# gnns4hri/3D_multi_pose_estimator

Measured on AMD Instinct MI355X. Metric: frames/sec (5-view Panoptic, 4 persons) at 1/2/4/8 GPUs; MPJPE vs ref, higher is better.
Workload: dtype f32

## Files before the change

### 3d_multi_pose_estimator_amd/csrc/api.hip

```cpp
#include <cmath>
#include <cstdarg>
#include <new>
#include <cstdio>
#include <cstdlib>
#include <cstring>

#include "mpe_internal.h"
#include "assign_int.h"

using namespace mpe;

namespace {

int fail(mpe_ctx *ctx, int code, const char *fmt, ...) {
    char buf[512];
    va_list ap;
    va_start(ap, fmt);
    vsnprintf(buf, sizeof buf, fmt, ap);
    va_end(ap);
    if (ctx) ctx->err = buf;
    return code;
}

#define HIPCHK(ctx, expr)                                                                     \
// ... 362 lines not shown
    const int V = ctx->cfg.n_cameras, J = ctx->cfg.n_joints, npj = ctx->cfg.numbers_per_joint;
    if (ctx->mlp[0].in_dim != V * J * npj)
        return fail(ctx, MPE_ERR_INVALID, "MLP input width %d != V*J*numbers_per_joint = %d", ctx->mlp[0].in_dim,
                    V * J * npj);
    int widest = 0;
    for (int l = 0; l < ctx->mlp_layers; ++l) {
        if (l > 0 && ctx->mlp[l].in_dim != ctx->mlp[l - 1].out_dim)
            return fail(ctx, MPE_ERR_INVALID, "MLP layer %d input width mismatch", l);
        widest = widest > ctx->mlp[l].out_dim ? widest : ctx->mlp[l].out_dim;
    }
    ctx->mlp_ld_in = round_up(ctx->mlp[0].in_dim, 128);
    ctx->mlp_ld_hidden = round_up(widest, 128);
    const size_t rows = (size_t)ctx->cfg.max_frames * ctx->cfg.max_persons_per_frame;
    int rc;
    if ((rc = dev_alloc(ctx, &ctx->mlp_rows, rows * ctx->mlp_ld_in))) return rc;
    for (int i = 0; i < 2; ++i)
        if ((rc = dev_alloc(ctx, &ctx->mlp_act[i], rows * ctx->mlp_ld_hidden))) return rc;
    ctx->mlp_ws_ready = true;
    return MPE_OK;
}

enum GatInput {
    GAT_IN_IMPLICIT,
    GAT_IN_DENSE0,
    GAT_IN_ACT
};

int gat_layer_linear(mpe_ctx *ctx, hipStream_t s, const mpe_batch *b, int l, GatInput in, AggArgs *a, int *n_rows_ft2) {
    GatLayer &g = ctx->gat[l];
    const int V = ctx->cfg.n_cameras, J = ctx->cfg.n_joints;
    const int n_nodes = b->n_heads + b->n_edge_nodes;
    const bool red = ctx->gat_reduced;
    const bool half_rows = red || ctx->gat_attn_fp16;
    const int ld_ft = half_rows ? 2 * ctx->act_ld : ctx->act_ld;
    int rc;
    const AttnCoef coef{g.attn_l, g.attn_r, ctx->a12, g.heads, g.out_dim};
    const bool no_epi = getenv("MPE_NO_COEF_EPILOGUE") != nullptr;
    const AttnCoef *cp = no_epi ? nullptr : &coef;
    bool done = false;
    if (in == GAT_IN_DENSE0) {
        if ((rc = gat_linear(ctx, s, ctx->xdense, ctx->feat_ld, g.fc1, ctx->hdense, ctx->feat_ld, n_nodes, nullptr,
                             true, ctx->gat_alpha, false)))
            return rc;
        if ((rc = gat_linear(ctx, s, ctx->hdense, ctx->feat_ld, g.fc2, ctx->act[2], ld_ft, n_nodes, nullptr, false,
                             0.f, half_rows, nullptr, nullptr, -1.0, cp, &done)))
            return rc;
        a->ft2 = ctx->act[2];
        *n_rows_ft2 = n_nodes;
    } else if (in == GAT_IN_IMPLICIT) {
        if (ctx->l0_grouped && !red && linear_uses_tile_kernel(b->n_heads, g.in_dim)) {
            GemmProf gp(ctx, s, 2.0 * b->n_heads * (double)g.in_dim * (J * 10), 0, 0);
            HIPCHK(ctx, launch_linear_grouped(s, ctx->xc, ctx->l0_ld, ctx->l0_w, ctx->l0_ld,
                                              (long)weight_rows(g.in_dim) * ctx->l0_ld, ctx->l0_b, ctx->h0, ctx->feat_ld,
                                              b->n_heads, ctx->cam_count, V, ctx->cam_list, ctx->cfg.max_heads, g.in_dim,
                                              ctx->l0_ld, true, ctx->gat_alpha, ctx->gat_acc64));
        } else if (ctx->l0_grouped) {
            const double flop_each = 2.0 * b->n_heads * (double)g.in_dim * (J * 10) / V;
            for (int c = 0; c < V; ++c)
                if ((rc = gat_linear(ctx, s, ctx->xc, ctx->l0_ld, ctx->l0_fc1[c], ctx->h0, ctx->feat_ld, b->n_heads,
                                     ctx->cam_count + c, true, ctx->gat_alpha, false,
                                     ctx->cam_list + (size_t)c * ctx->cfg.max_heads,
                                     ctx->cam_list + (size_t)c * ctx->cfg.max_heads, flop_each)))
                    return rc;
        } else if ((rc = gat_linear(ctx, s, ctx->x0, ctx->feat_ld, g.fc1, ctx->h0, ctx->feat_ld, b->n_heads, nullptr,
                                    true, ctx->gat_alpha, false)))
            return rc;
        if ((rc = gat_linear(ctx, s, ctx->h0, ctx->feat_ld, g.fc2, ctx->act[1], ld_ft, b->n_heads, nullptr, false,
                             0.f, half_rows, nullptr, nullptr, -1.0, cp, &done)))
            return rc;
        a->ft2 = ctx->act[1];
        *n_rows_ft2 = b->n_heads;
        a->en_const_ft2 = ctx->en0_ft2;
        a->en_const_a = ctx->en0_a;
    } else {
        if ((rc = gat_linear(ctx, s, ctx->act[0], ctx->act_ld, g.fc1, ctx->act[1], ctx->act_ld, n_nodes, nullptr,
                             true, ctx->gat_alpha, false)))
            return rc;
        if ((rc = gat_linear(ctx, s, ctx->act[1], ctx->act_ld, g.fc2, ctx->act[2], ld_ft, n_nodes, nullptr, false,
                             0.f, half_rows, nullptr, nullptr, -1.0, cp, &done)))
            return rc;
        a->ft2 = ctx->act[2];
        *n_rows_ft2 = n_nodes;
    }
    if (!done && cp && g.out_dim == 40 && !half_rows && ctx->gat_split && !red) {
        HIPCHK(ctx, launch_attn_coef(s, a->ft2, ld_ft, *n_rows_ft2, g.heads, g.out_dim, g.attn_l, g.attn_r, ctx->a12, 0));
        done = true;
    }
    a->a12_ready = done ? 1 : 0;
    return MPE_OK;
}

AggArgs gat_agg_args(const mpe_ctx *ctx, int l) {
    const GatLayer &g = ctx->gat[l];
    AggArgs a{};
    a.heads = g.heads;
    a.out_dim = g.out_dim;
    a.alpha = ctx->gat_alpha;
    a.out_slope = ctx->gat_hidden_slope;
    const bool half_rows = ctx->gat_reduced || ctx->gat_attn_fp16;
    a.ft_half = half_rows ? 1 : 0;
    a.ld = half_rows ? 2 * ctx->act_ld : ctx->act_ld;
    a.a12 = ctx->a12;
    return a;
}

void agg_scores_out(const mpe_ctx *ctx, AggArgs *a, float *d_scores_en, float *d_scores_heads) {
    a->out_mode = ctx->gat_out_mode;
    a->score_mode = 1;
    a->out = d_scores_en;
    a->out_heads = d_scores_heads;
    a->ld_out = 1;
}

int gat_attention(mpe_ctx *ctx, hipStream_t s, const mpe_batch *b, int l, const AggArgs &a, int n_rows_ft2) {
    const GatLayer &g = ctx->gat[l];
    HIPCHK(ctx, launch_gat_attention(s, *b, ctx->cfg.n_cameras, ctx->cfg.max_heads_per_frame, ctx->node_off,
                                     ctx->head_frame, ctx->en_frame, ctx->en_pair, g.attn_l, g.attn_r, ctx->a12, a,
                                     n_rows_ft2, ctx->head_src, explicit_deg_cap(ctx->cfg.max_heads_per_frame), ctx->x_m_cap));
    return MPE_OK;
}

int gat_topology(mpe_ctx *ctx, hipStream_t s, const mpe_batch *b) {
    if (b->d_en_pair && (size_t)b->n_frames * ctx->cfg.max_heads_per_frame * explicit_deg_cap(ctx->cfg.max_heads_per_frame) > ctx->head_src_cap)
        return fail(ctx, MPE_ERR_CAPACITY, "in-edge table too small for %d frames with explicit edge-node lists", b->n_frames);
    HIPCHK(ctx, launch_topology(s, *b, ctx->cfg.n_cameras, ctx->node_off, ctx->head_frame, ctx->en_frame, ctx->en_pair,
                                ctx->cfg.max_heads_per_frame, ctx->d_status, ctx->head_src,
                                explicit_deg_cap(ctx->cfg.max_heads_per_frame), ctx->x_m_cap));
    return MPE_OK;
}

constexpr int LAT_MAX_FRAMES = 16;
constexpr int LAT_MAX_NODES = 16384;

bool lat_gat_ok(mpe_ctx *ctx, const mpe_batch *b, bool dense_in) {
    if (!latency_path_on() || dense_in || b->d_en_pair || b->n_frames > LAT_MAX_FRAMES) return false;
    if (b->n_heads + b->n_edge_nodes > LAT_MAX_NODES || b->n_heads <= 0) return false;
    if (!ctx->gat_split || ctx->gat_acc64 || ctx->gat_reduced || ctx->gat_attn_fp16 || !ctx->l0_grouped) return false;
    if (getenv("MPE_NO_COEF_EPILOGUE") || getenv("MPE_GAT_ACC64_MINK") || getenv("MPE_SKINNY_WAVES") || getenv("MPE_GEMM_NARROW")) return false;
    if (!lat_l0a_available(ctx->cfg.n_joints, ctx->l0_ld)) return false;
    const GatLayer &g0 = ctx->gat[0];
    if (g0.out_dim != 40 || g0.in_dim <= 512) return false;
    for (int l = 1; l < ctx->gat_layers; ++l) {
        const GatLayer &g = ctx->gat[l];
        if (!lat_gemm_available(g.fc1.ldw, g.in_dim, false, 0) || !lat_gemm_available(g.fc2.ldw, g.heads * g.out_dim, true, g.out_dim)) return false;
        if (g.in_dim > 512) return false;
    }
    const size_t shm = (size_t)2 * ((size_t)16 * (ctx->cfg.max_heads_per_frame + 1) + (ctx->cfg.max_heads_per_frame + 1) + 1 +
                                    (size_t)(ctx->cfg.n_cameras + 1) * (ctx->cfg.n_cameras + 1)) * sizeof(float);
    return shm <= 40 * 1024;
}

int ensure_lat_workspace(mpe_ctx *ctx) {
    if (ctx->gat_pl[0]) return MPE_OK;
    ctx->lat_rows = ctx->max_nodes < LAT_MAX_NODES ? ctx->max_nodes : LAT_MAX_NODES;
    ctx->gat_pl_plane = (size_t)ctx->lat_rows * ctx->act_ld;
    int rc;
    for (int i = 0; i < 2; ++i)
        if ((rc = dev_alloc(ctx, &ctx->gat_pl[i], 3 * ctx->gat_pl_plane))) return rc;
    return MPE_OK;
}

struct LatTail {
    bool deferred = false;
    const float *ft2 = nullptr;
    int ld = 0;
    float alpha = 0.f, out_slope = 0.f;
    int out_mode = 0;
// ... 1601 lines not shown
```

### 3d_multi_pose_estimator_amd/csrc/gat.hip

```cpp
#include <cstdlib>

#include "mpe_internal.h"
#include "sb_common.h"

namespace mpe {

__device__ __forceinline__ void topology_body(int f, int n_frames, int V, const int32_t *__restrict__ head_off,
                                              const int32_t *__restrict__ en_off, const int32_t *__restrict__ slot_n,
                                              int32_t *__restrict__ node_off, int32_t *__restrict__ head_frame,
                                              int32_t *__restrict__ en_frame, int32_t *__restrict__ en_pair, int hmax,
                                              int32_t *__restrict__ status) {
    __shared__ int s_n[MPE_MAX_CAMERAS], s_start[MPE_MAX_CAMERAS];
    const int h0 = head_off[f], H = head_off[f + 1] - h0;
    const int e0 = en_off[f], M = en_off[f + 1] - e0;
    if (threadIdx.x == 0) {
        int acc = 0;
        for (int s = 0; s < V; ++s) {
            s_n[s] = slot_n[f * V + s];
            s_start[s] = acc;
            acc += s_n[s];
        }
        node_off[f] = h0 + e0;
        if (H > hmax && status) atomicOr(status, 1);
        if (f == n_frames - 1) node_off[n_frames] = head_off[n_frames] + en_off[n_frames];
    }
    __syncthreads();
    for (int i = threadIdx.x; i < H; i += blockDim.x) head_frame[h0 + i] = f;
    for (int i = threadIdx.x; i < M; i += blockDim.x) en_frame[e0 + i] = f;
    int base = 0;
    for (int a = 0; a < V; ++a)
        for (int b = a + 1; b < V; ++b) {
            const int na = s_n[a], nb = s_n[b], cnt = na * nb;
            for (int t = threadIdx.x; t < cnt; t += blockDim.x) {
                const int i = t / nb, j = t - i * nb;
                en_pair[2 * (size_t)(e0 + base + t) + 0] = s_start[a] + i;
                en_pair[2 * (size_t)(e0 + base + t) + 1] = s_start[b] + j;
            }
            base += cnt;
        }
}

__global__ void k_topology(int n_frames, int V, const int32_t *__restrict__ head_off,
                           const int32_t *__restrict__ en_off, const int32_t *__restrict__ slot_n,
                           int32_t *__restrict__ node_off, int32_t *__restrict__ head_frame,
                           int32_t *__restrict__ en_frame, int32_t *__restrict__ en_pair, int hmax,
                           int32_t *__restrict__ status) {
    topology_body(blockIdx.x, n_frames, V, head_off, en_off, slot_n, node_off, head_frame, en_frame, en_pair, hmax, status);
}

__global__ void k_head_sources(int V, int hmax, const int32_t *__restrict__ head_off,
                               const int32_t *__restrict__ slot_n, uint16_t *__restrict__ head_src);

size_t head_src_entries(int max_heads_per_frame, int V) {
    const size_t h = (size_t)max_heads_per_frame;
    const size_t nodes = h + h * h * (size_t)(V - 1) / (2 * (size_t)V) + 1;
    return nodes <= 65535 ? h * (h + 1) : 0;
}

constexpr int XT_CHUNK = 2048;
__global__ __launch_bounds__(256) void k_topology_explicit(int n_frames, const int32_t *__restrict__ head_off,
                                                           const int32_t *__restrict__ en_off,
                                                           const int32_t *__restrict__ pairs_in,
                                                           int32_t *__restrict__ node_off, int32_t *__restrict__ head_frame,
                                                           int32_t *__restrict__ en_frame, int32_t *__restrict__ en_pair,
                                                           uint16_t *__restrict__ head_src, int hmax, int deg_cap, int m_cap,
                                                           int32_t *__restrict__ status) {
    __shared__ uint32_t s_pr[XT_CHUNK];
    const int f = blockIdx.x, t = threadIdx.x;
    const int h0 = head_off[f], H = head_off[f + 1] - h0;
    const int e0 = en_off[f], M = en_off[f + 1] - e0;
    const bool ok = H <= hmax && M <= m_cap;
    if (t == 0) {
        node_off[f] = h0 + e0;
        if (f == n_frames - 1) node_off[n_frames] = head_off[n_frames] + en_off[n_frames];
        if (!ok && status) atomicOr(status, 1);
    }
    for (int i = t; i < H; i += blockDim.x) head_frame[h0 + i] = f;
    int flag = 0;
    uint16_t *tab = head_src + (size_t)f * hmax * deg_cap;
    int deg_a[4];
#pragma unroll
    for (int r = 0; r < 4; ++r) {
        const int h = t + r * 256;
        deg_a[r] = 0;
// ... 605 lines not shown
            }
#pragma unroll
            for (int j = 0; j < 4; ++j)
#pragma unroll
                for (int k = 0; k < VEC; ++k) {
                    const float m = fv[j][k] * w[j];
                    acc[hf * 4 + j][k] = acc[hf * 4 + j][k] + m;
                }
        }
    }
#pragma unroll
    for (int j = 0; j < 8; ++j)
        if (e + j < deg) {
            float fv[VEC];
            row(e + j, fv);
            const float w = wt(e + j);
#pragma unroll
            for (int k = 0; k < VEC; ++k) {
                const float m = fv[k] * w;
                acc[j][k] = acc[j][k] + m;
            }
        }
#pragma unroll
    for (int k = 0; k < VEC; ++k)
        out[k] = ((acc[0][k] + acc[1][k]) + (acc[2][k] + acc[3][k])) + ((acc[4][k] + acc[5][k]) + (acc[6][k] + acc[7][k]));
}

constexpr int EN_ROWS = 16;

template <int VEC>
__device__ __forceinline__ void agg_store_row(const AggArgs &a, size_t row, int c, const float *o) {
    if (a.out_pl) {
        unsigned short *d = a.out_pl + row * a.ld_out + c;
        if (VEC == 4) {
            sb::f32x4 v = {o[0], o[1], o[2], o[3]};
            sb::store_planes4(d, a.out_pl_plane, v);
        } else {
#pragma unroll
            for (int k = 0; k < VEC; ++k) sb::store_planes1(d + k, a.out_pl_plane, o[k]);
        }
        return;
    }
    typedef float vecf __attribute__((ext_vector_type(VEC)));
    vecf v;
#pragma unroll
    for (int k = 0; k < VEC; ++k) v[k] = o[k];
    *reinterpret_cast<vecf *>(a.out + row * a.ld_out + c) = v;
}

__device__ __forceinline__ void row_coef(const float *__restrict__ fv, const AggArgs &a, int hh, float &x1, float &x2) {
    const float *al = a.attn_l + hh * a.out_dim, *ar = a.attn_r + hh * a.out_dim;
    if (a.out_dim == 40) {
        float v[40];
#pragma unroll
        for (int q = 0; q < 10; ++q) {
            const float4 x = *reinterpret_cast<const float4 *>(fv + 4 * q);
            v[4 * q] = x.x;
            v[4 * q + 1] = x.y;
            v[4 * q + 2] = x.z;
            v[4 * q + 3] = x.w;
        }
        coef40([&](int d) { return v[d]; }, al, ar, hh & 1, x1, x2);
    } else if (a.out_dim == 30) {
        float v[30];
#pragma unroll
        for (int q = 0; q < 15; ++q) {
            const float2 x = *reinterpret_cast<const float2 *>(fv + 2 * q);
            v[2 * q] = x.x;
            v[2 * q + 1] = x.y;
        }
        x1 = x2 = 0.f;
#pragma unroll
        for (int d = 0; d < 30; ++d) {
            x1 = __builtin_fmaf(v[d], al[d], x1);
            x2 = __builtin_fmaf(v[d], ar[d], x2);
        }
    } else {
        x1 = x2 = 0.f;
        for (int d = 0; d < a.out_dim; ++d) {
            x1 = __builtin_fmaf(fv[d], al[d], x1);
            x2 = __builtin_fmaf(fv[d], ar[d], x2);
        }
    }
}

template <int VEC, int ER = 16>
__device__ __forceinline__ void aggregate_en_body(int wg, int n_en, const int32_t *__restrict__ head_off,
                                                  const int32_t *__restrict__ en_off,
                                                  const int32_t *__restrict__ node_off,
                                                  const int32_t *__restrict__ en_frame,
                                                  const int32_t *__restrict__ en_pair, const AggArgs &a, int hmax) {
#pragma clang fp contract(off)
    __shared__ float s_w[ER][16][3];
    __shared__ int s_over[ER];
    __shared__ long s_src[ER][3];
    __shared__ long s_dst[ER];
    const int hd = a.heads * a.out_dim, heads = a.heads;
    const int per_row = (hd + VEC - 1) / VEC;
    const int m0 = wg * ER;
    const int rows = min(ER, n_en - m0);
    const bool l0 = a.en_const_ft2 != nullptr;
    for (int i = threadIdx.x; i < rows * heads; i += blockDim.x) {
        const int r = i / heads, hh = i - r * heads;
        const int m = m0 + r;
        const int f = en_frame[m];
        const int hb = head_off[f], H = head_off[f + 1] - hb;
        const int nb = node_off[f];
        const int v = H + (m - en_off[f]);
        const int h1 = en_pair[2 * (size_t)m], h2 = en_pair[2 * (size_t)m + 1];
        const float *ra1, *ra2, *ra3;
        if (l0) {
            ra1 = a.a12 + (size_t)(hb + h1) * 32;
            ra2 = a.a12 + (size_t)(hb + h2) * 32;
            ra3 = a.en_const_a;
        } else {
            ra1 = a.a12 + (size_t)(nb + h1) * 32;
            ra2 = a.a12 + (size_t)(nb + h2) * 32;
            ra3 = a.a12 + (size_t)(nb + v) * 32;
        }
        float a2v, c1, c2, c3;
        if (a.a12_ready) {
            a2v = ra3[16 + hh];
            c1 = ra1[hh];
            c2 = ra2[hh];
            c3 = ra3[hh];
        } else {
            const size_t rb = (size_t)(l0 ? hb : nb);
            float unused;
            row_coef(a.ft2 + (rb + h1) * a.ld + hh * a.out_dim, a, hh, c1, unused);
            row_coef(a.ft2 + (rb + h2) * a.ld + hh * a.out_dim, a, hh, c2, unused);
            if (l0) {
                c3 = a.en_const_a[hh];
                a2v = a.en_const_a[16 + hh];
            } else {
                row_coef(a.ft2 + (rb + v) * a.ld + hh * a.out_dim, a, hh, c3, a2v);
            }
        }
        float e1 = c1 + a2v, e2 = c2 + a2v, e3 = c3 + a2v;
        e1 = e1 > 0.f ? e1 : e1 * a.alpha;
        e2 = e2 > 0.f ? e2 : e2 * a.alpha;
        e3 = e3 > 0.f ? e3 : e3 * a.alpha;
        const float mx = fmaxf(fmaxf(e1, e2), e3);
        const float x1 = expf(e1 - mx), x2 = expf(e2 - mx), x3 = expf(e3 - mx);
        const float sum = (x1 + x2) + x3;
        s_w[r][hh][0] = x1 / sum;
        s_w[r][hh][1] = x2 / sum;
        s_w[r][hh][2] = x3 / sum;
        if (hh == 0) {
            s_src[r][0] = (long)(l0 ? hb : nb) + h1;
            s_src[r][1] = (long)(l0 ? hb : nb) + h2;
            s_src[r][2] = l0 ? -1 : (long)nb + v;
            s_dst[r] = (long)nb + v;
            s_over[r] = H > hmax ? 1 : 0;
        }
    }
    __syncthreads();
    for (int i = threadIdx.x; i < rows * per_row; i += blockDim.x) {
        const int r = i / per_row;
        const int c = (i - r * per_row) * VEC;
        const int hh = c / a.out_dim;
        float v1[VEC], v2[VEC], v3[VEC];
        ld_ftv<VEC>(a.ft2, (size_t)s_src[r][0] * a.ld + c, a.ft_half, v1);
        ld_ftv<VEC>(a.ft2, (size_t)s_src[r][1] * a.ld + c, a.ft_half, v2);
        if (l0) ld_ftv<VEC>(a.en_const_ft2, (size_t)c, 0, v3);
        else ld_ftv<VEC>(a.ft2, (size_t)s_src[r][2] * a.ld + c, a.ft_half, v3);
        float w1[VEC], w2[VEC], w3[VEC];
        const bool one_head = VEC == 1 || (c + VEC <= hd && (c + VEC - 1) / a.out_dim == hh);
#pragma unroll
        for (int k = 0; k < VEC; ++k) {
            int hk = hh;
            if (!one_head) {
                hk = (c + k) / a.out_dim;
                hk = hk < heads ? hk : heads - 1;
            }
            w1[k] = s_w[r][hk][0];
            w2[k] = s_w[r][hk][1];
            w3[k] = s_w[r][hk][2];
        }
        float o[VEC];
#pragma unroll
        for (int k = 0; k < VEC; ++k) {
            float acc = v1[k] * w1[k];
            acc = acc + v2[k] * w2[k];
            acc = acc + v3[k] * w3[k];
            o[k] = agg_activate(acc, a.out_mode, a.out_slope);
        }
        if (a.score_mode) a.out[m0 + r] = s_over[r] ? 0.f : o[0];
        else agg_store_row<VEC>(a, (size_t)s_dst[r], c, o);
    }
}

template <int VEC>
__global__ __launch_bounds__(256) void k_aggregate_en(int n_en, const int32_t *__restrict__ head_off,
                                                      const int32_t *__restrict__ en_off,
                                                      const int32_t *__restrict__ node_off,
                                                      const int32_t *__restrict__ en_frame,
                                                      const int32_t *__restrict__ en_pair, AggArgs a, int hmax) {
    aggregate_en_body<VEC, EN_ROWS>(blockIdx.x, n_en, head_off, en_off, node_off, en_frame, en_pair, a, hmax);
}

constexpr int AGG_ROWS = 2;

template <int VEC>
__device__ __forceinline__ void aggregate_heads_body(
    int wg, float *s_dyn, int n_heads, int V, int max_deg, const int32_t *__restrict__ head_off, const int32_t *__restrict__ en_off,
    const int32_t *__restrict__ slot_n, const int32_t *__restrict__ node_off,
    const int32_t *__restrict__ head_frame, const AggArgs &a, const uint16_t *__restrict__ head_src, int src_stride, int hmax) {
#pragma clang fp contract(off)
    const int heads = a.heads, hd = a.heads * a.out_dim;
    float *s_w = s_dyn;
    int *s_src = reinterpret_cast<int *>(s_w + (size_t)AGG_ROWS * heads * max_deg);
    int *s_topo = s_src + AGG_ROWS * max_deg;
    __shared__ int s_deg[AGG_ROWS], s_f[AGG_ROWS], s_v[AGG_ROWS], s_H[AGG_ROWS];

    const int t = threadIdx.x, lane = t & 63, wave = t >> 6;
    const bool l0 = a.en_const_ft2 != nullptr;
    const int r_own = wave & (AGG_ROWS - 1), half = wave / AGG_ROWS;
    const int gh = wg * AGG_ROWS + r_own;
    int deg = 0, f = 0, hb = 0, H = 0, v = 0;
    int32_t nb = 0;
    const int32_t *sn = slot_n;
    FrameTopo tp;
    tp.start = s_topo + r_own * (V + 1 + V * V);
    tp.base = tp.start + V + 1;
    bool live = false;
    if (gh < n_heads) {
        f = head_frame[gh];
        hb = head_off[f];
        H = head_off[f + 1] - hb;
        live = H <= hmax;
// ... 469 lines not shown
                    }
                    *reinterpret_cast<vecf *>(dst + 4 * g) = o;
                }
            } else {
                const int node = i / DV, d = (i - node * DV) * VEC;
                const int deg = s_deg[node];
                const int *src = s_src + node * max_deg;
                const float *w = s_wh + node * max_deg;
                float acc[VEC];
                weighted_sum8<VEC>(
                    deg,
                    [&](int e, float *fv) {
                        const vecf x = *reinterpret_cast<const vecf *>(s_ft + src[e] * Dp + d);
#pragma unroll
                        for (int k = 0; k < VEC; ++k) fv[k] = x[k];
                    },
                    [&](int e) { return w[e]; }, acc);
                vecf o;
#pragma unroll
                for (int k = 0; k < VEC; ++k) o[k] = agg_activate(acc[k], a.out_mode, a.out_slope);
                *reinterpret_cast<vecf *>(a.out + (size_t)(nb + node) * a.ld_out + c0 + d) = o;
            }
        }
        FUSED_STAMP(3);
        return;
    }
    for (int i = first * DV + t; i < N * DV; i += blockDim.x) {
        const int node = i / DV, d = (i - node * DV) * VEC;
        vecf o;
        if (node >= H) {
            const int m = node - H;
            const int pr = s_pair[m];
            const int h1 = pr >> 16, h2 = pr & 0xFFFF;
            const float w1 = s_wen[m * 3 + 0], w2 = s_wen[m * 3 + 1], w3 = s_wen[m * 3 + 2];
            const vecf f1 = *reinterpret_cast<const vecf *>(s_ft + h1 * Dp + d);
            const vecf f2 = *reinterpret_cast<const vecf *>(s_ft + h2 * Dp + d);
            const vecf f3 = *reinterpret_cast<const vecf *>(s_ft + node * Dp + d);
#pragma unroll
            for (int k = 0; k < VEC; ++k) {
                float acc = f1[k] * w1;
                acc = acc + f2[k] * w2;
                acc = acc + f3[k] * w3;
                o[k] = agg_activate(acc, a.out_mode, a.out_slope);
            }
        } else {
            const int deg = s_deg[node];
            const int *src = s_src + node * max_deg;
            const float *w = s_wh + node * max_deg;
            float acc[VEC];
            weighted_sum8<VEC>(
                deg,
                [&](int e, float *fv) {
                    const vecf x = *reinterpret_cast<const vecf *>(s_ft + src[e] * Dp + d);
#pragma unroll
                    for (int k = 0; k < VEC; ++k) fv[k] = x[k];
                },
                [&](int e) { return w[e]; }, acc);
#pragma unroll
            for (int k = 0; k < VEC; ++k) o[k] = agg_activate(acc[k], a.out_mode, a.out_slope);
        }
        if (a.score_mode) {
            if (node >= H) a.out[(size_t)eb + (node - H)] = o[0];
            else a.out_heads[(size_t)hb + node] = o[0];
        } else {
            *reinterpret_cast<vecf *>(a.out + (size_t)(nb + node) * a.ld_out + c0 + d) = o;
        }
    }
    FUSED_STAMP(3);
}

#ifdef MPE_FUSED_CLOCK
}
extern "C" int mpe_debug_fused_stamps(unsigned int *out, int clear) {
    if (hipMemcpyFromSymbol(out, HIP_SYMBOL(mpe::g_fused_stamp), sizeof(mpe::g_fused_stamp)) != hipSuccess) return -1;
    if (clear) {
        void *p = nullptr;
        if (hipGetSymbolAddress(&p, HIP_SYMBOL(mpe::g_fused_stamp)) != hipSuccess || hipMemset(p, 0, sizeof(mpe::g_fused_stamp)) != hipSuccess) return -1;
    }
    return 0;
}
namespace mpe {
#endif

static size_t fused_lds_bytes(int hmax, int V, int out_dim, int *n_cap, int *m_cap, int *max_deg, int x_deg_cap, int x_m_cap) {
    const int mc = x_m_cap > 0 ? x_m_cap : hmax * hmax * (V - 1) / (2 * V) + 1;
    const int nc = hmax + mc;
    const int deg = x_m_cap > 0 ? x_deg_cap : hmax + 1;
    const int Dp = out_dim;
    size_t image = (size_t)nc * Dp + 256;
    if (out_dim % 4 == 0 && image < (size_t)FUSED_PIECES * 1024)
        image = (size_t)FUSED_PIECES * 1024;
    const size_t bytes = (fused_tables_floats(hmax, deg, V, nc, mc) + image) * sizeof(float);
    *n_cap = nc;
    *m_cap = mc;
    *max_deg = deg;
    return bytes;
}

static int agg_vec(const AggArgs &a) {
    if (!a.score_mode && a.ld % 4 == 0 && a.ld_out % 4 == 0) {
        if (a.out_dim % 4 == 0) return 4;
        if (a.out_dim % 2 == 0) return 2;
    }
    return 1;
}

static bool half_vec8() {
    static const bool v = !(getenv("MPE_HALF_VEC") && atoi(getenv("MPE_HALF_VEC")) == 4);
    return v;
}

constexpr size_t FUSED_LDS_LIMIT = 160 * 1024;

hipError_t launch_gat_attention(hipStream_t s, const mpe_batch &b, int V, int max_heads_per_frame,
                                const int32_t *node_off, const int32_t *head_frame, const int32_t *en_frame,
                                const int32_t *en_pair, const float *attn_l, const float *attn_r, float *a12,
                                const AggArgs &a, int n_rows_ft2, const uint16_t *head_src, int x_deg_cap, int x_m_cap) {
    int n_cap, m_cap, max_deg;
    const bool xpl = b.d_en_pair != nullptr;
    if (xpl && (!head_src || x_m_cap <= 0)) return hipErrorInvalidValue;
    if (!xpl) x_deg_cap = x_m_cap = 0;
    if (!xpl && getenv("MPE_NO_HEAD_SRC_TABLE")) head_src = nullptr;
    const size_t shm = fused_lds_bytes(max_heads_per_frame, V, a.out_dim, &n_cap, &m_cap, &max_deg, x_deg_cap, x_m_cap);
    const bool no_fuse = getenv("MPE_NO_FUSED_ATTENTION") != nullptr;
    if (shm <= FUSED_LDS_LIMIT && !no_fuse && b.n_frames > 0) {
        const int vec = agg_vec(a);
        const int grp = max_deg <= 32 ? 16 : max_deg <= 64 ? 32 : 64;
        if (!xpl && !head_src_entries(max_heads_per_frame, V)) head_src = nullptr;
        const int overlap = ((!xpl && vec == 4 && a.a12_ready && !a.ft_half && n_cap <= 256 && m_cap <= 256 && head_src &&
                              max_heads_per_frame * (max_heads_per_frame + 1) <= 512 &&
                              n_cap * (a.out_dim / 4) <= FUSED_PIECES * 256 && !getenv("MPE_FUSED_NO_OVERLAP")) ? 1 : 0) |
                            (getenv("MPE_FUSED_NO_OVERLAP") ? 2 : 0);
        const void *fn = nullptr;
#define MPE_FUSED(V_, G_)                                                                                     \
    do {                                                                                                      \
        fn = reinterpret_cast<const void *>(k_gat_fused<V_, G_>);                                             \
        if (shm > 64 * 1024) {                                                                                \
            hipError_t e_ = hipFuncSetAttribute(fn, hipFuncAttributeMaxDynamicSharedMemorySize, (int)FUSED_LDS_LIMIT); \
            if (e_ != hipSuccess) return e_;                                                                  \
        }                                                                                                     \
        hipLaunchKernelGGL((k_gat_fused<V_, G_>), dim3(b.n_frames * a.heads), dim3(256), shm, s, V,            \
                           max_deg, max_heads_per_frame, n_cap, m_cap, b.d_frame_head_off, b.d_frame_en_off, b.d_slot_n, \
                           node_off, en_pair, attn_l, attn_r, a, overlap, head_src);                          \
    } while (0)
#define MPE_FUSED_G(V_)                     \
    do {                                    \
        if (grp == 16) MPE_FUSED(V_, 16);   \
        else if (grp == 32) MPE_FUSED(V_, 32); \
        else MPE_FUSED(V_, 64);             \
    } while (0)
        if (vec == 4) MPE_FUSED_G(4);
        else if (vec == 2) MPE_FUSED_G(2);
        else MPE_FUSED_G(1);
#undef MPE_FUSED_G
#undef MPE_FUSED
        return hipGetLastError();
    }
    AggArgs a2 = a;
    a2.a12 = a12;
    if (!a.a12_ready) {
        hipError_t e = launch_attn_coef(s, a.ft2, a.ld, n_rows_ft2, a.heads, a.out_dim, attn_l, attn_r, a12, a.ft_half);
        if (e != hipSuccess) return e;
        a2.a12_ready = 1;
    }
    return launch_aggregate(s, b, V, max_heads_per_frame, node_off, head_frame, en_frame, en_pair, a2, head_src, x_deg_cap);
}

hipError_t launch_lat_attention(hipStream_t s, const mpe_batch &b, int V, int max_heads_per_frame, const int32_t *node_off,
                                const int32_t *head_frame, const int32_t *en_frame, const int32_t *en_pair, const AggArgs &a,
                                const uint16_t *head_src) {
    if (b.d_en_pair || a.ft_half || (!a.a12_ready && (!a.attn_l || !a.attn_r))) return hipErrorInvalidValue;
    const int vec = agg_vec(a);
    if (!head_src_entries(max_heads_per_frame, V)) head_src = nullptr;
    const int n_en_wgs = (b.n_edge_nodes + LAT_EN_ROWS - 1) / LAT_EN_ROWS;
    const bool heads_on = b.n_heads > 0 && (!a.score_mode || a.out_heads);
    const int n_h_wgs = heads_on ? (b.n_heads + AGG_ROWS - 1) / AGG_ROWS : 0;
    if (n_en_wgs + n_h_wgs == 0) return hipSuccess;
    const int src_stride = max_heads_per_frame + 1;
    int max_deg = src_stride < 3 ? 3 : src_stride;
    const size_t shm = (size_t)AGG_ROWS * ((size_t)a.heads * max_deg + max_deg + (V + 1) + (size_t)V * V + 16) * sizeof(float);
    if (shm > 48 * 1024) return hipErrorInvalidValue;
    const int hd4 = (a.heads * a.out_dim + 3) / 4 * 4;
    (void)hd4;
#define MPE_LA(V_)                                                                                                              \
    hipLaunchKernelGGL(k_lat_attention<V_>, dim3(n_en_wgs + n_h_wgs), dim3(256), shm, s, n_en_wgs, b.n_edge_nodes, b.n_heads, V, max_deg, \
                       b.d_frame_head_off, b.d_frame_en_off, b.d_slot_n, node_off, head_frame, en_frame, en_pair, a, head_src, src_stride, \
                       max_heads_per_frame)
    if (vec == 4) MPE_LA(4);
    else if (vec == 2) MPE_LA(2);
    else MPE_LA(1);
#undef MPE_LA
    return hipGetLastError();
}

hipError_t launch_aggregate(hipStream_t s, const mpe_batch &b, int V, int max_heads_per_frame,
                            const int32_t *node_off, const int32_t *head_frame, const int32_t *en_frame,
                            const int32_t *en_pair, const AggArgs &a, const uint16_t *head_src, int x_deg_cap) {
    const int vec = agg_vec(a);
    const bool xpl = b.d_en_pair != nullptr;
    if (xpl && (!head_src || x_deg_cap <= 0)) return hipErrorInvalidValue;
    if (!xpl && !head_src_entries(max_heads_per_frame, V)) head_src = nullptr;
    if (b.n_edge_nodes > 0) {
        const unsigned blocks = (unsigned)((b.n_edge_nodes + EN_ROWS - 1) / EN_ROWS);
#define MPE_EN(V_)                                                                                      \
// ... 46 lines not shown
```

### 3d_multi_pose_estimator_amd/csrc/mpe_internal.h

```cpp
#pragma once
#include <hip/hip_runtime.h>
#include <stdint.h>
#include <string>
#include <vector>

#include "../../include/mpe.h"
#include "gemm_form.h"

namespace mpe {

constexpr int GEMM_BM = 128;
constexpr int GEMM_BN = 80;
constexpr int GEMM_BK = 32;
constexpr int GEMM_BN_MAX = 208;
inline int weight_rows(int out_dim) { return (out_dim + 15) / 16 * 16 + GEMM_BN_MAX; }
constexpr int LD_ALIGN = 32;

inline int round_up(int x, int m) { return (x + m - 1) / m * m; }

struct Linear {
    float *w = nullptr;
    float *b = nullptr;
    unsigned short *w16 = nullptr;
    int ldw16 = 0;
// ... 207 lines not shown
struct DecodeEpi {
    const int32_t *person_off;
    int n_frames, pcap, n_out;
    float scale;
    float *poses;
};
hipError_t launch_linear_sb16(hipStream_t s, const float *A, int lda, const unsigned short *W3, size_t w_plane, int ldw,
                              const float *bias, float *C, int ldc, int m_cap, const int32_t *d_m, int n, int k_pad, bool leaky,
                              float slope, bool f64 = true, const AttnCoef *coef = nullptr, bool *coef_done = nullptr,
                              bool out_half = false,
                              int flush_stages = 2,
                              const DecodeEpi *dec = nullptr, bool *dec_done = nullptr);
bool linear_sb16_uses_tile_kernel(int m_cap, int n, bool f64);
int device_cu_count();

bool lat_gemm_available(int k_pad, int n, bool fc2, int out_dim);
hipError_t launch_lat_gemm(hipStream_t s, const unsigned short *Apl, int lda, size_t a_plane, const unsigned short *W3, size_t w_plane, int ldw,
                           const float *bias, float *C, int ldc, unsigned short *Cpl, int ldcp, size_t c_plane, int m, int n, int k_pad, bool fc2,
                           float slope, const float *attn_l, const float *attn_r, float *a12, int out_dim, bool *coef_done = nullptr);
bool lat_gemm_fusable(int k1_pad, int n1, int k2_pad, int n2, int out_dim2);
hipError_t launch_lat_gemm_fused(hipStream_t s, const unsigned short *Apl, int lda, size_t a_plane, const unsigned short *W3, size_t w_plane, int ldw,
                                 const float *bias, int m, int n, float slope, const unsigned short *W3b, size_t w_plane_b, int ldw_b, const float *bias_b,
                                 float *C2, int ldc2, const float *attn_l, const float *attn_r, float *a12);
hipError_t launch_linear_f64(hipStream_t s, const float *A, int lda, const float *W, int ldw, const float *bias, float *C, int ldc,
                             int m_cap, const int32_t *d_m, int n, int k_pad, bool leaky, float slope);
hipError_t launch_linear(hipStream_t s, const float *A, int lda, const float *W, int ldw, const float *bias,
                         float *C, int ldc, int m_cap, const int32_t *d_m, int n, int k_pad, bool leaky,
                         float slope, bool acc64, const int32_t *a_rows = nullptr, const int32_t *c_rows = nullptr,
                         const AttnCoef *coef = nullptr, bool *coef_done = nullptr, bool out_half = false);
hipError_t launch_linear_grouped(hipStream_t s, const float *A, int lda, const float *W, int ldw, long w_grp_stride,
                                 const float *bias, float *C, int ldc, int m_cap, const int32_t *grp_count, int n_grp,
                                 const int32_t *row_lists, int grp_stride, int n, int k_pad, bool leaky, float slope, bool acc64 = false);
bool linear_uses_tile_kernel(int m_cap, int n);
hipError_t launch_onehot_rows(hipStream_t s, float *rows, int n_rows, int ld, int col);
hipError_t launch_group_heads(hipStream_t s, int n_heads, int V, const int32_t *head_cam, int32_t *cam_count,
                              int32_t *cam_list, int list_stride, bool counts_zeroed = false);

hipError_t launch_linear_bf16(hipStream_t s, const float *A, int lda, const unsigned short *Wb, int ldw,
                              const float *bias, float *C, int ldc, int m_cap, const int32_t *d_m, int n, int k_pad,
                              bool leaky, float slope, int k_lim = 0, bool out_half = false,
                              const int32_t *a_rows = nullptr, const int32_t *c_rows = nullptr);

hipError_t launch_split_planes(hipStream_t s, const float *w, size_t count, unsigned short *planes);
hipError_t launch_topology(hipStream_t s, const mpe_batch &b, int V, int32_t *node_off, int32_t *head_frame,
                           int32_t *en_frame, int32_t *en_pair, int max_heads_per_frame, int32_t *status,
                           uint16_t *head_src, int x_deg_cap = 0, int x_m_cap = 0);
inline int explicit_deg_cap(int max_heads_per_frame) { return 2 * max_heads_per_frame; }
size_t head_src_entries(int max_heads_per_frame, int V);
hipError_t launch_head_features(hipStream_t s, const DevCfg *cfg, const mpe_batch &b, int J, float *feat,
                                int ld_feat, int col0, int stride_cam, bool dense, int32_t *zero_counts = nullptr,
                                int n_zero = 0);
hipError_t launch_attn_coef(hipStream_t s, const float *ft2, int ld, int n_rows, int heads, int out_dim,
                            const float *attn_l, const float *attn_r, float *a12, int ft_half = 0);
struct AggArgs {
    const float *ft2;
    int ld;
    int ft_half;
    const float *a12;
    int a12_ready;
    int heads, out_dim;
    float alpha, out_slope;
    int out_mode;
    const float *en_const_ft2;
    const float *en_const_a;
    float *out;
    int ld_out;
    int score_mode;
    float *out_heads;
    const float *attn_l, *attn_r;
    unsigned short *out_pl;
    size_t out_pl_plane;
};
hipError_t launch_aggregate(hipStream_t s, const mpe_batch &b, int V, int max_heads_per_frame,
                            const int32_t *node_off, const int32_t *head_frame, const int32_t *en_frame,
                            const int32_t *en_pair, const AggArgs &a, const uint16_t *head_src, int x_deg_cap = 0);

bool lat_l0a_available(int J, int l0_ld);
hipError_t launch_lat_l0a(hipStream_t s, const DevCfg *cfg, const mpe_batch &b, int V, int J, int32_t *node_off, int32_t *head_frame,
                          int32_t *en_frame, int32_t *en_pair, uint16_t *head_src, int hmax, int32_t *status, const float *l0_w,
                          long w_cam_stride, int l0_ld, const float *l0_b, int n_out, float *h0, int ld_h0, float alpha);
hipError_t launch_lat_attention(hipStream_t s, const mpe_batch &b, int V, int max_heads_per_frame, const int32_t *node_off,
                                const int32_t *head_frame, const int32_t *en_frame, const int32_t *en_pair, const AggArgs &a,
                                const uint16_t *head_src);
hipError_t launch_gat_attention(hipStream_t s, const mpe_batch &b, int V, int max_heads_per_frame,
                                const int32_t *node_off, const int32_t *head_frame, const int32_t *en_frame,
                                const int32_t *en_pair, const float *attn_l, const float *attn_r, float *a12,
                                const AggArgs &a, int n_rows_ft2, const uint16_t *head_src, int x_deg_cap = 0,
                                int x_m_cap = 0);

size_t cluster_keys_per_frame(int max_heads_per_frame);
size_t cluster_scratch_per_frame(int max_heads_per_frame);
hipError_t launch_cluster(hipStream_t s, const DevCfg *cfg, const mpe_batch &b, const int32_t *en_pair,
                          const float *scores, int pcap, int max_heads_per_frame, uint64_t *keys,
                          size_t keys_per_frame, int32_t *scratch, size_t scratch_per_frame,
                          int32_t *persons, int32_t *n_persons);

bool lat_tail_available(int hmax, size_t keys_per_frame);
hipError_t launch_lat_tail(hipStream_t s, const DevCfg *cfg, const mpe_batch &b, int J, const int32_t *en_pair, const int32_t *en_frame,
                           const float *ft2, int ld, const float *a12, float alpha, float out_slope, int out_mode, const int32_t *node_off,
                           float *scores, int pcap, int hmax, size_t keys_per_frame, int32_t *persons, int32_t *n_persons, double *pair_pts);

hipError_t launch_person_scan(hipStream_t s, int n_frames, int pcap, const int32_t *n_persons, int32_t *person_off,
                              int32_t *total);
hipError_t launch_mlp_rows(hipStream_t s, const DevCfg *cfg, int V, int J, const mpe_batch &b,
                           const int32_t *persons, const int32_t *n_persons, const int32_t *person_off, int pcap,
                           float *rows, int ld_rows, uint8_t *valid, int32_t *scan_out = nullptr, int32_t *total_out = nullptr,
                           float *zero_poses = nullptr, int n_out = 0, const double *pair_pts = nullptr, int pair_hmax = 0);

hipError_t launch_triangulate(hipStream_t s, const DevCfg *cfg, int V, int J, const mpe_batch &b,
                              const int32_t *persons, const int32_t *n_persons, int pcap, double *poses,
                              uint8_t *joint_valid, uint32_t out_mask, bool positive_ids_only = false);
hipError_t launch_dlt_pairs(hipStream_t s, const DevCfg *cfg, const double *pts, const int32_t *cams, int n,
                            double *out);
hipError_t launch_decode(hipStream_t s, int n_frames, int pcap, int n_out, float scale, const int32_t *n_persons,
                         const int32_t *person_off, const float *y, int ld_y, float *poses);
int cluster_table_cap(int hmax);

hipError_t launch_eval(hipStream_t s, const mpe_eval_args &a);

hipError_t track_prepare(int pcap);
hipError_t launch_track_reset(hipStream_t s, mpe_track_state *st);
hipError_t launch_track(hipStream_t s, mpe_track_state *st, const mpe_track_args &a);

hipError_t launch_smooth_reset(hipStream_t s, mpe_smooth_state *st);
hipError_t launch_smooth(hipStream_t s, mpe_smooth_state *st, const mpe_smooth_args &a);

void skel_schedule(const int32_t *bones, int n_bones, std::vector<uint32_t> *table, int *steps_upto);
hipError_t launch_skel_reset(hipStream_t s, mpe_skel_state *st);
hipError_t launch_skel_observe(hipStream_t s, mpe_skel_state *st, const mpe_skel_args &a);
hipError_t launch_skel_update(hipStream_t s, mpe_skel_state *st, int min_samples);
hipError_t launch_skel_fit(hipStream_t s, mpe_skel_state *st, const mpe_skel_args &a);

hipError_t launch_track_score_reset(hipStream_t s, mpe_track_score_state *st);
hipError_t launch_track_score(hipStream_t s, mpe_track_score_state *st, const mpe_track_score_args &a);

hipError_t launch_reproject(hipStream_t s, const DevCfg *cfg, int V, const mpe_batch &b, const mpe_reproject_args &a);
hipError_t launch_refine(hipStream_t s, const DevCfg *cfg, int V, const mpe_batch &b, const mpe_refine_args &a);
size_t calib_workspace_doubles(int max_frames, int V);
hipError_t launch_calib(hipStream_t s, const DevCfg *cfg, int V, mpe_calib_state *st, const mpe_batch &b, const mpe_calib_args &a);
hipError_t launch_calib_clear(hipStream_t s, mpe_calib_state *st, int V);
constexpr size_t GEOM_LDS_BYTES = 48 * 1024;
bool geom_needs_table(int max_heads_per_frame, int J);
size_t geom_table_doubles(int max_heads, int J);
hipError_t launch_geom(hipStream_t s, const DevCfg *cfg, int V, int J, const mpe_batch &b, const int32_t *en_pair, int max_heads_per_frame,
                       int x_m_cap, const mpe_geom_args &a, float *scores, double *ray_table);
hipError_t launch_partition_labels(hipStream_t s, int V, const mpe_batch &b, const mpe_partition_labels_args &a);
hipError_t launch_group_bodies(hipStream_t s, const mpe_group_bodies_args &a);
hipError_t launch_partition_scores(hipStream_t s, const mpe_partition_scores_args &a, const double *log_table, int n_log);
hipError_t launch_residual_stats(hipStream_t s, int V, const mpe_residual_stats_args &a, ResidualState *state, uint32_t *hist,
                                 double *partial);

}
```

Measured before the change: 272,800.

## Add row-slab fused GAT layer-0 attention kernel using implicit edge-node constants

```diff
diff --git a/3d_multi_pose_estimator_amd/csrc/api.hip b/3d_multi_pose_estimator_amd/csrc/api.hip
--- a/3d_multi_pose_estimator_amd/csrc/api.hip
+++ b/3d_multi_pose_estimator_amd/csrc/api.hip
@@ -468,7 +468,9 @@
         a->ft2 = ctx->act[2];
         *n_rows_ft2 = n_nodes;
     }
-    if (!done && cp && g.out_dim == 40 && !half_rows && ctx->gat_split && !red) {
+    const bool l0_rows = in == GAT_IN_IMPLICIT && l < ctx->gat_layers - 1 &&
+                         gat_l0_rows_available(*b, V, ctx->cfg.max_heads_per_frame, g.heads, g.out_dim, half_rows ? 1 : 0, ld_ft, ctx->head_src);
+    if (!done && cp && g.out_dim == 40 && !half_rows && ctx->gat_split && !red && !l0_rows) {
         HIPCHK(ctx, launch_attn_coef(s, a->ft2, ld_ft, *n_rows_ft2, g.heads, g.out_dim, g.attn_l, g.attn_r, ctx->a12, 0));
         done = true;
     }
diff --git a/3d_multi_pose_estimator_amd/csrc/gat.hip b/3d_multi_pose_estimator_amd/csrc/gat.hip
--- a/3d_multi_pose_estimator_amd/csrc/gat.hip
+++ b/3d_multi_pose_estimator_amd/csrc/gat.hip
@@ -1,5 +1,6 @@
 #include <cstdlib>
 
+#include "gat_l0_rows.h"
 #include "mpe_internal.h"
 #include "sb_common.h"
 
@@ -771,6 +772,20 @@
             x2 = __builtin_fmaf(fv[d], ar[d], x2);
         }
     }
+}
+
+__device__ __forceinline__ void en_softmax3(float c1, float c2, float c3, float a2v, float alpha, float *w) {
+#pragma clang fp contract(off)
+    float e1 = c1 + a2v, e2 = c2 + a2v, e3 = c3 + a2v;
+    e1 = e1 > 0.f ? e1 : e1 * alpha;
+    e2 = e2 > 0.f ? e2 : e2 * alpha;
+    e3 = e3 > 0.f ? e3 : e3 * alpha;
+    const float mx = fmaxf(fmaxf(e1, e2), e3);
+    const float x1 = expf(e1 - mx), x2 = expf(e2 - mx), x3 = expf(e3 - mx);
+    const float sum = (x1 + x2) + x3;
+    w[0] = x1 / sum;
+    w[1] = x2 / sum;
+    w[2] = x3 / sum;
 }
 
 template <int VEC, int ER = 16>
@@ -825,16 +840,7 @@
                 row_coef(a.ft2 + (rb + v) * a.ld + hh * a.out_dim, a, hh, c3, a2v);
             }
         }
-        float e1 = c1 + a2v, e2 = c2 + a2v, e3 = c3 + a2v;
-        e1 = e1 > 0.f ? e1 : e1 * a.alpha;
-        e2 = e2 > 0.f ? e2 : e2 * a.alpha;
-        e3 = e3 > 0.f ? e3 : e3 * a.alpha;
-        const float mx = fmaxf(fmaxf(e1, e2), e3);
-        const float x1 = expf(e1 - mx), x2 = expf(e2 - mx), x3 = expf(e3 - mx);
-        const float sum = (x1 + x2) + x3;
-        s_w[r][hh][0] = x1 / sum;
-        s_w[r][hh][1] = x2 / sum;
-        s_w[r][hh][2] = x3 / sum;
+        en_softmax3(c1, c2, c3, a2v, a.alpha, s_w[r][hh]);
         if (hh == 0) {
             s_src[r][0] = (long)(l0 ? hb : nb) + h1;
             s_src[r][1] = (long)(l0 ? hb : nb) + h2;
@@ -1470,6 +1476,189 @@
 namespace mpe {
 #endif
 
+template <int G>
+__global__ __launch_bounds__(L0R_THREADS) void k_gat_l0_rows(int max_deg, int hmax, int n_cap, int m_cap, int slabs, int head_rows, int en_rows,
+                                                     const int32_t *__restrict__ head_off, const int32_t *__restrict__ en_off,
+                                                     const int32_t *__restrict__ node_off, const int32_t *__restrict__ en_pair,
+                                                     const float *__restrict__ attn_l, const float *__restrict__ attn_r, AggArgs a,
+                                                     const uint16_t *__restrict__ head_src) {
+#pragma clang fp contract(off)
+    typedef float vecf __attribute__((ext_vector_type(4)));
+    extern __shared__ __attribute__((aligned(1024))) float s_dyn[];
+    const int bid = blockIdx.x, nwg = gridDim.x;
+    const int xcd = bid & 7, xq = nwg >> 3, xr = nwg & 7;
+    const int vid = (xcd < xr ? xcd * (xq + 1) : xr * (xq + 1) + (xcd - xr) * xq) + (bid >> 3);
+    const int f = vid / slabs, sl = vid - f * slabs;
+    const int heads = a.heads, hd = heads * 40, per_row = hd / 4;
+    const int hb = head_off[f], H = head_off[f + 1] - hb;
+    const int eb = en_off[f], M = en_off[f + 1] - eb;
+    const int N = H + M, nb = node_off[f];
+    if (M <= 0) return;
+    if (H > hmax || N > n_cap || M > m_cap) return;
+    const int per_slab = (N + slabs - 1) / slabs;
+    const int lo = sl * per_slab, hi = min(N, lo + per_slab);
+    if (lo >= hi) return;
+    const L0RowsLayout L = l0_rows_layout(hmax, heads, 40, max_deg, head_rows, en_rows);
+    float *s_ft = s_dyn + L.ft;
+    float *s_a1 = s_dyn + L.a1, *s_a2 = s_dyn + L.a2;
+    float *s_wh = s_dyn + L.wh;
+    int *s_src = reinterpret_cast<int *>(s_dyn + L.src);
+    int *s_deg = reinterpret_cast<int *>(s_dyn + L.deg);
+    float *s_wen = s_dyn + L.wen;
+    int *s_pair = reinterpret_cast<int *>(s_dyn + L.pair);
+    const int t = threadIdx.x;
+    constexpr int NT = L0R_THREADS;
+
+    const int total = H * per_row;
+    for (int i0 = t; i0 < total; i0 += 4 * NT) {
+        vecf v[4];
+#pragma unroll
+        for (int u = 0; u < 4; ++u) {
+            int i = i0 + u * NT;
+            i = i < total ? i : total - 1;
+            const int r = i / per_row, d = (i - r * per_row) * 4;
+            v[u] = *reinterpret_cast<const vecf *>(a.ft2 + (size_t)(hb + r) * a.ld + d);
+        }
+#pragma unroll
+        for (int u = 0; u < 4; ++u) {
+            const int i = i0 + u * NT;
+            if (i < total) *reinterpret_cast<vecf *>(s_ft + (size_t)i * 4) = v[u];
+        }
+    }
+    __syncthreads();
+    for (int i = t; i < (H + 1) * heads; i += NT) {
+        const int r = i / heads, hh = i - r * heads;
+        float x1, x2;
+        if (r < H) {
+            const float *fv = s_ft + r * hd + hh * 40;
+            float v[40];
+#pragma unroll
+            for (int q = 0; q < 10; ++q) {
+                const vecf x = *reinterpret_cast<const vecf *>(fv + 4 * q);
+                v[4 * q] = x[0];
+                v[4 * q + 1] = x[1];
+                v[4 * q + 2] = x[2];
+                v[4 * q + 3] = x[3];
+            }
+            coef40([&](int d) { return v[d]; }, attn_l + hh * 40, attn_r + hh * 40, hh & 1, x1, x2);
+        } else {
+            x1 = a.en_const_a[hh];
+            x2 = a.en_const_a[16 + hh];
+        }
+        s_a1[i] = x1;
+        s_a2[i] = x2;
+    }
+    __syncthreads();
+
+    const int tcols = per_row < NT ? per_row : NT;
+    const int rps = NT / tcols;
+    const int r_in = t / tcols, c_in = t - r_in * tcols;
+    const bool active = r_in < rps;
+    for (int row0 = lo; row0 < hi;) {
+        int n;
+        if (row0 < H) {
+            n = min(head_rows, min(H, hi) - row0);
+            const uint16_t *tab = head_src + ((size_t)f * hmax + row0) * max_deg;
+            for (int i = t; i < n * max_deg; i += NT) {
+                const int u = tab[i];
+                s_src[i] = u == 0xFFFF ? -1 : u;
+            }
+            __syncthreads();
+            const int gl = t & (G - 1);
+            for (int j = t / G; j < n * heads; j += NT / G) {
+                const int r = j / heads, hh = j - r * heads;
+                float *w = s_wh + (size_t)j * max_deg;
+                const int *src = s_src + r * max_deg;
+                const float a2v = s_a2[(row0 + r) * heads + hh];
+                float mx = -INFINITY;
+                int deg = 0;
+                for (int e = gl; e < max_deg; e += G) {
+                    const int u = src[e];
+                    if (u >= 0) {
+                        float x = s_a1[(u < H ? u : H) * heads + hh] + a2v;
+                        x = x > 0.f ? x : x * a.alpha;
+                        w[e] = x;
+                        mx = fmaxf(mx, x);
+                        deg = e + 1;
+                    }
+                }
+                mx = group_max<G>(mx);
+                deg = (int)group_max<G>((float)deg);
+                float sum = 0.f;
+                for (int e = gl; e < deg; e += G) {
+                    const float ex = expf(w[e] - mx);
+                    w[e] = ex;
+                    sum = sum + ex;
+                }
+                sum = group_sum<G>(sum);
+                for (int e = gl; e < deg; e += G) w[e] = w[e] / sum;
+                if (gl == 0 && hh == 0) s_deg[r] = deg;
+            }
+            __syncthreads();
+            if (active)
+                for (int c = c_in; c < per_row; c += tcols) {
+                    const int hh = c / 10;
+                    const vecf f3 = *reinterpret_cast<const vecf *>(a.en_const_ft2 + 4 * c);
+                    for (int r = r_in; r < n; r += rps) {
+                        const int deg = s_deg[r];
+                        const int *src = s_src + r * max_deg;
+                        const float *w = s_wh + (size_t)(r * heads + hh) * max_deg;
+                        float acc[4];
+                        weighted_sum8<4>(
+                            deg,
+                            [&](int e, float *fv) {
+                                const int u = src[e];
+                                vecf x = f3;
+                                if (u < H) x = *reinterpret_cast<const vecf *>(s_ft + u * hd + 4 * c);
+#pragma unroll
+                                for (int k = 0; k < 4; ++k) fv[k] = x[k];
+                            },
+                            [&](int e) { return w[e]; }, acc);
+                        vecf o;
+#pragma unroll
+                        for (int k = 0; k < 4; ++k) o[k] = agg_activate(acc[k], a.out_mode, a.out_slope);
+                        *reinterpret_cast<vecf *>(a.out + (size_t)(nb + row0 + r) * a.ld_out + 4 * c) = o;
+                    }
+                }
+        } else {
+            n = min(en_rows, hi - row0);
+            for (int i = t; i < n * heads; i += NT) {
+                const int r = i / heads, hh = i - r * heads;
+                const size_t m = (size_t)eb + (row0 + r - H);
+                const int h1 = en_pair[2 * m], h2 = en_pair[2 * m + 1];
+                en_softmax3(s_a1[h1 * heads + hh], s_a1[h2 * heads + hh], s_a1[H * heads + hh], s_a2[H * heads + hh], a.alpha,
+                            s_wen + (size_t)i * 3);
+                if (hh == 0) s_pair[r] = (h1 << 16) | h2;
+            }
+            __syncthreads();
+            if (active)
+                for (int c = c_in; c < per_row; c += tcols) {
+                    const int hh = c / 10;
+                    const vecf f3 = *reinterpret_cast<const vecf *>(a.en_const_ft2 + 4 * c);
+                    for (int r = r_in; r < n; r += rps) {
+                        const int pr = s_pair[r];
+                        const int h1 = pr >> 16, h2 = pr & 0xFFFF;
+                        const float *w = s_wen + (size_t)(r * heads + hh) * 3;
+                        const float w1 = w[0], w2 = w[1], w3 = w[2];
+                        const vecf f1 = *reinterpret_cast<const vecf *>(s_ft + h1 * hd + 4 * c);
+                        const vecf f2 = *reinterpret_cast<const vecf *>(s_ft + h2 * hd + 4 * c);
+                        vecf o;
+#pragma unroll
+                        for (int k = 0; k < 4; ++k) {
+                            float acc = f1[k] * w1;
+                            acc = acc + f2[k] * w2;
+                            acc = acc + f3[k] * w3;
+                            o[k] = agg_activate(acc, a.out_mode, a.out_slope);
+                        }
+                        *reinterpret_cast<vecf *>(a.out + (size_t)(nb + row0 + r) * a.ld_out + 4 * c) = o;
+                    }
+                }
+        }
+        row0 += n;
+        if (row0 < hi) __syncthreads();
+    }
+}
+
 static size_t fused_lds_bytes(int hmax, int V, int out_dim, int *n_cap, int *m_cap, int *max_deg, int x_deg_cap, int x_m_cap) {
     const int mc = x_m_cap > 0 ? x_m_cap : hmax * hmax * (V - 1) / (2 * V) + 1;
     const int nc = hmax + mc;
@@ -1500,6 +1689,48 @@
 
 constexpr size_t FUSED_LDS_LIMIT = 160 * 1024;
 
+bool gat_l0_rows_available(const mpe_batch &b, int V, int max_heads_per_frame, int heads, int out_dim, int ft_half, int ld,
+                           const uint16_t *head_src) {
+    if (b.d_en_pair || b.n_frames <= 0 || !head_src || !head_src_entries(max_heads_per_frame, V)) return false;
+    if (ft_half || out_dim != 40 || heads < 1 || heads > 16 || ld % 4 != 0 || heads * 40 > ld) return false;
+    if (getenv("MPE_NO_FUSED_ATTENTION") || getenv("MPE_NO_HEAD_SRC_TABLE")) return false;
+    const char *sw = getenv("MPE_L0_ROW_ATTENTION");
+    if (sw && atoi(sw) == 0) return false;
+    const int m_cap = max_heads_per_frame * max_heads_per_frame * (V - 1) / (2 * V) + 1;
+    return l0_rows_plan(max_heads_per_frame, heads, 40, max_heads_per_frame + 1, m_cap).fits;
+}
+
+static hipError_t launch_gat_l0_rows(hipStream_t s, const mpe_batch &b, int V, int hmax, const int32_t *node_off,
+                                     const int32_t *en_pair, const float *attn_l, const float *attn_r, const AggArgs &a,
+                                     const uint16_t *head_src) {
+    int n_cap, m_cap, max_deg;
+    (void)fused_lds_bytes(hmax, V, a.out_dim, &n_cap, &m_cap, &max_deg, 0, 0);
+    const L0RowsPlan pl = l0_rows_plan(hmax, a.heads, 40, max_deg, m_cap);
+    if (!pl.fits) return hipErrorInvalidValue;
+    const size_t shm = pl.lds_bytes;
+    if (shm > 64 * 1024) {
+        static PerDeviceFlag attr;
+        if (!attr.test()) {
+            hipError_t e = hipSuccess;
+            const void *fns[3] = {reinterpret_cast<const void *>(k_gat_l0_rows<16>), reinterpret_cast<const void *>(k_gat_l0_rows<32>),
+                                  reinterpret_cast<const void *>(k_gat_l0_rows<64>)};
+            for (const void *fn : fns)
+                if (e == hipSuccess) e = hipFuncSetAttribute(fn, hipFuncAttributeMaxDynamicSharedMemorySize, (int)FUSED_LDS_LIMIT);
+            if (e != hipSuccess) return e;
+            attr.set();
+        }
+    }
+    const int grp = max_deg <= 32 ? 16 : max_deg <= 64 ? 32 : 64;
+#define MPE_L0R(G_)                                                                                                                  \
+    hipLaunchKernelGGL(k_gat_l0_rows<G_>, dim3(b.n_frames * pl.slabs), dim3(L0R_THREADS), shm, s, max_deg, hmax, n_cap, m_cap, pl.slabs, \
+                       pl.head_rows, pl.en_rows, b.d_frame_head_off, b.d_frame_en_off, node_off, en_pair, attn_l, attn_r, a, head_src)
+    if (grp == 16) MPE_L0R(16);
+    else if (grp == 32) MPE_L0R(32);
+    else MPE_L0R(64);
+#undef MPE_L0R
+    return hipGetLastError();
+}
+
 hipError_t launch_gat_attention(hipStream_t s, const mpe_batch &b, int V, int max_heads_per_frame,
                                 const int32_t *node_off, const int32_t *head_frame, const int32_t *en_frame,
                                 const int32_t *en_pair, const float *attn_l, const float *attn_r, float *a12,
@@ -1508,6 +1739,9 @@
     const bool xpl = b.d_en_pair != nullptr;
     if (xpl && (!head_src || x_m_cap <= 0)) return hipErrorInvalidValue;
     if (!xpl) x_deg_cap = x_m_cap = 0;
+    if (a.en_const_ft2 && a.en_const_a && !a.score_mode && !a.out_pl && a.out && a.ld_out % 4 == 0 && a.heads * 40 <= a.ld_out &&
+        gat_l0_rows_available(b, V, max_heads_per_frame, a.heads, a.out_dim, a.ft_half, a.ld, head_src))
+        return launch_gat_l0_rows(s, b, V, max_heads_per_frame, node_off, en_pair, attn_l, attn_r, a, head_src);
     if (!xpl && getenv("MPE_NO_HEAD_SRC_TABLE")) head_src = nullptr;
     const size_t shm = fused_lds_bytes(max_heads_per_frame, V, a.out_dim, &n_cap, &m_cap, &max_deg, x_deg_cap, x_m_cap);
     const bool no_fuse = getenv("MPE_NO_FUSED_ATTENTION") != nullptr;
diff --git a/3d_multi_pose_estimator_amd/csrc/gat_l0_rows.h b/3d_multi_pose_estimator_amd/csrc/gat_l0_rows.h
--- /dev/null
+++ b/3d_multi_pose_estimator_amd/csrc/gat_l0_rows.h
@@ -0,0 +1,82 @@
+#pragma once
+#include <stddef.h>
+
+#if defined(__HIPCC__)
+#define MPE_L0R_HD __host__ __device__
+#else
+#define MPE_L0R_HD
+#endif
+
+namespace mpe {
+
+#ifndef MPE_L0R_THREADS
+#define MPE_L0R_THREADS 512
+#endif
+constexpr int L0R_THREADS = MPE_L0R_THREADS;
+constexpr int L0R_SLAB_ROWS = 512;
+constexpr int L0R_MAX_SLABS = 8;
+constexpr int L0R_HEAD_ROWS = 24;
+constexpr int L0R_EN_ROWS = 256;
+constexpr size_t L0R_LDS_LIMIT = 160 * 1024;
+
+struct L0RowsLayout {
+    size_t ft;
+    size_t a1;
+    size_t a2;
+    size_t wh;
+    size_t src;
+    size_t deg;
+    size_t wen;
+    size_t pair;
+    size_t total;
+};
+
+MPE_L0R_HD inline L0RowsLayout l0_rows_layout(int hmax, int heads, int out_dim, int max_deg, int head_rows, int en_rows) {
+    L0RowsLayout l;
+    size_t o = 0;
+    l.ft = o;
+    o += (size_t)hmax * heads * out_dim;
+    l.a1 = o;
+    o += (size_t)(hmax + 1) * heads;
+    l.a2 = o;
+    o += (size_t)(hmax + 1) * heads;
+    o = (o + 3) & ~(size_t)3;
+    l.wh = o;
+    o += (size_t)head_rows * heads * max_deg;
+    l.src = o;
+    o += (size_t)head_rows * max_deg;
+    l.deg = o;
+    o += head_rows;
+    l.wen = o;
+    o += (size_t)en_rows * heads * 3;
+    l.pair = o;
+    o += en_rows;
+    l.total = (o + 255) & ~(size_t)255;
+    return l;
+}
+
+struct L0RowsPlan {
+    int slabs, head_rows, en_rows;
+    size_t lds_bytes;
+    bool fits;
+};
+
+inline L0RowsPlan l0_rows_plan(int hmax, int heads, int out_dim, int max_deg, int m_cap) {
+    L0RowsPlan p;
+    const int n_cap = hmax + m_cap;
+    p.slabs = (n_cap + L0R_SLAB_ROWS - 1) / L0R_SLAB_ROWS;
+    p.slabs = p.slabs < 1 ? 1 : p.slabs > L0R_MAX_SLABS ? L0R_MAX_SLABS : p.slabs;
+    p.head_rows = hmax < L0R_HEAD_ROWS ? hmax : L0R_HEAD_ROWS;
+    p.en_rows = m_cap < L0R_EN_ROWS ? m_cap : L0R_EN_ROWS;
+    for (;;) {
+        p.lds_bytes = l0_rows_layout(hmax, heads, out_dim, max_deg, p.head_rows, p.en_rows).total * sizeof(float);
+        if (p.lds_bytes <= L0R_LDS_LIMIT) break;
+        if (p.en_rows > 32) p.en_rows = (p.en_rows + 1) / 2;
+        else if (p.head_rows > 4) p.head_rows = (p.head_rows + 1) / 2;
+        else break;
+    }
+    p.fits = p.lds_bytes <= L0R_LDS_LIMIT;
+    return p;
+}
+
+}
diff --git a/3d_multi_pose_estimator_amd/csrc/mpe_internal.h b/3d_multi_pose_estimator_amd/csrc/mpe_internal.h
--- a/3d_multi_pose_estimator_amd/csrc/mpe_internal.h
+++ b/3d_multi_pose_estimator_amd/csrc/mpe_internal.h
@@ -313,6 +313,8 @@
 hipError_t launch_lat_attention(hipStream_t s, const mpe_batch &b, int V, int max_heads_per_frame, const int32_t *node_off,
                                 const int32_t *head_frame, const int32_t *en_frame, const int32_t *en_pair, const AggArgs &a,
                                 const uint16_t *head_src);
+bool gat_l0_rows_available(const mpe_batch &b, int V, int max_heads_per_frame, int heads, int out_dim, int ft_half, int ld,
+                           const uint16_t *head_src);
 hipError_t launch_gat_attention(hipStream_t s, const mpe_batch &b, int V, int max_heads_per_frame,
                                 const int32_t *node_off, const int32_t *head_frame, const int32_t *en_frame,
                                 const int32_t *en_pair, const float *attn_l, const float *attn_r, float *a12,
```

Measured after the change: 270,900. No clear change (-0.7%).
